# zzyunzhi/object-intrinsics

Measured on AMD Instinct MI355X. Metric: rendered rays/sec (64x64 img, 128 samples/ray) + D-images/sec, higher is better.
Workload: dtype f32 via f16x3 (fp32 operands split into 2 fp16 limbs = 22 mantissa bits, 3 fp16 MFMAs per product, fp32 accumulate: 2^-22 relative per product, 1e-4 parity path); 1 GPU; C2: 1x64x64 crop per GPU, 64+64 samples/ray, 1 up-sampling step(s), Generator.forward (render + Phong maps) + ADADiscriminatorView forward; parallelism=dp1 (independent renders, no data-path collective)

## Files before the change

object-intrinsics_amd/csrc/mlp_fwd3.hip:

```cpp
#include <type_traits>

#include "mlp_common.h"
#include "f3_blob.h"

namespace {

using namespace oimlp;
static_assert(oif3::FC == C && oif3::HB_SIG == H_SIG && oif3::HB_TABS_END == H_TABS_END && oif3::HB_BIAS == H_BIAS &&
              oif3::HB_WSCALE == H_WSCALE && oif3::HB_NL_SDF == NL_SDF, "f3_blob.h mirrors the packed header's offsets");

constexpr int F3_WAVES = 4;
constexpr int F3_TILE = F3_WAVES * WAVE_PTS;
using oif3::F3_FILM;
using oif3::F3_FILM_ROW;
using oif3::F3_TABS;
using oif3::F3_GMAX;
using oif3::F3_BLOB;
constexpr int F3_LDS = F3_BLOB + 2 * 65536;

typedef float Bank[16][4];
__device__ __forceinline__ float to_acc(float v) {
  float a;
  asm("v_accvgpr_write_b32 %0, %1" : "=a"(a) : "v"(v));
  return a;
}
__device__ __forceinline__ float from_acc(float a) {
  float v;
  asm("v_accvgpr_read_b32 %0, %1" : "=v"(v) : "a"(a));
  return v;
}

constexpr int F3_CU_SLOTS = 4096;
constexpr int F3_WG_SLOTS = 512;
__device__ __forceinline__ int cu_slot_id() {
  const unsigned xcc = __builtin_amdgcn_s_getreg((4 - 1) << 11 | 0 << 6 | 20);
  const unsigned cu = __builtin_amdgcn_s_getreg((8 - 1) << 11 | 8 << 6 | 4);
  return (int)(xcc * 256 + cu);
}

typedef float f32x2 __attribute__((ext_vector_type(2)));
__device__ __forceinline__ f32x2 pk_fma(f32x2 a, f32x2 b, f32x2 c) {
  return __builtin_elementwise_fma(a, b, c);
}
__device__ __forceinline__ f32x2 pk_mul(f32x2 a, f32x2 b) {
  return a * b;
}
__device__ __forceinline__ f32x2 pk_mul_s(f32x2 a, float s) {
  return a * s;
}
__device__ __forceinline__ f32x2 film_phase2(const f32x4& a, const f32x4& b, int k, float acc0, float acc1) {
  return pk_fma(f32x2{a[k], a[k + 1]}, f32x2{acc0, acc1}, f32x2{b[k], b[k + 1]});
}
__device__ __forceinline__ float max3_abs(float m, float x, float y) {
  float r;
  asm("v_max3_f32 %0, %1, |%2|, |%3|" : "=v"(r) : "v"(m), "v"(x), "v"(y));
  return r;
}

typedef unsigned Limbs[8][4];


__device__ __forceinline__ void split_limbs_normalised(const float (&act)[64], float m, float& run, Limbs& bh, Limbs& bl) {
  m = fmaxf(m, __shfl_xor(m, 32, 64));
  int eb = (__builtin_bit_cast(int, m) >> 23) & 0xff;
  eb = eb < 14 ? 14 : (eb > 254 ? 254 : eb);
  const float sc = __builtin_bit_cast(float, (267 - eb) << 23);
  run *= __builtin_bit_cast(float, (eb - 13) << 23);
#pragma unroll
  for (int s = 0; s < 8; ++s) {
#pragma unroll
    for (int d = 0; d < 4; ++d) split_pair(act[8 * s + 2 * d] * sc, act[8 * s + 2 * d + 1] * sc, bh[s][d], bl[s][d]);
    __builtin_amdgcn_sched_barrier(0);
  }
}
__device__ __forceinline__ void split_limbs(const float (&act)[64], Limbs& bh, Limbs& bl) {
#pragma unroll
  for (int s = 0; s < 8; ++s) {
#pragma unroll
    for (int d = 0; d < 4; ++d) split_pair(act[8 * s + 2 * d], act[8 * s + 2 * d + 1], bh[s][d], bl[s][d]);
    __builtin_amdgcn_sched_barrier(0);
  }
}

struct NoTail {
  __device__ __forceinline__ void operator()(int, int) const {}
};
template <class T> struct is_no_tail { static constexpr bool value = false; };
template <> struct is_no_tail<NoTail> { static constexpr bool value = true; };

constexpr int F3_ADIST = 1;
constexpr int F3_VALU_PER_MFMA = 6;
struct NoMid {
  __device__ __forceinline__ void operator()() const {}
};
template <class TAIL, class MID, class EPI>
__device__ __forceinline__ void stream_layer(const char* lds, const LayOff& y, const Limbs& bh, const Limbs& bl,
                                             f32x16 (&acc)[4], TAIL&& tail, MID&& mid, EPI&& epi) {
  constexpr bool HAS_TAIL = !is_no_tail<std::remove_cv_t<std::remove_reference_t<TAIL>>>::value;
  constexpr int AD = F3_ADIST;
  f32x4 ah[AD + 1], al[AD + 1];
#pragma unroll
  for (int i = 0; i < AD; ++i) {
    ah[i] = lds_f4(lds, i * 1024, y.wl);
    al[i] = lds_f4(lds, i * 1024, y.wh);
  }
#pragma unroll
  for (int t = 0; t < 4; ++t) {
#pragma unroll
    for (int r = 0; r < 16; ++r) acc[t][r] = 0.f;
#pragma unroll
    for (int s = 0; s < 8; ++s) {
      const int cur = t * 8 + s, nxt = cur + AD;
      if (nxt < 32) {
        ah[nxt % (AD + 1)] = lds_f4(lds, nxt * 1024, y.wl);
        al[nxt % (AD + 1)] = lds_f4(lds, nxt * 1024, y.wh);
      }
      int npairs = 0;
      if (t == 0) {
        if (HAS_TAIL && s < 6) {
          constexpr int first[7] = {0, 2, 3, 4, 6, 7, 8};
          for (int rp = first[s]; rp < first[s + 1]; ++rp) tail(3, rp);
          npairs = first[s + 1] - first[s];
        }
      } else {
        epi(t - 1, s);
        npairs = 1;
      }
      const int ci = cur % (AD + 1);
      const f16x8 wh = __builtin_bit_cast(f16x8, ah[ci]);
      const f16x8 wl = __builtin_bit_cast(f16x8, al[ci]);
      const u32x4 uh = {bh[s][0], bh[s][1], bh[s][2], bh[s][3]}, ul = {bl[s][0], bl[s][1], bl[s][2], bl[s][3]};
      const f16x8 vh = __builtin_bit_cast(f16x8, uh);
      const f16x8 vl = __builtin_bit_cast(f16x8, ul);
      acc[t] = __builtin_amdgcn_mfma_f32_32x32x16_f16(wl, vh, acc[t], 0, 0, 0);
      acc[t] = __builtin_amdgcn_mfma_f32_32x32x16_f16(wh, vl, acc[t], 0, 0, 0);
      acc[t] = __builtin_amdgcn_mfma_f32_32x32x16_f16(wh, vh, acc[t], 0, 0, 0);
      if (npairs >= 1) {
#pragma unroll
        for (int q = 0; q < 2; ++q) {
          __builtin_amdgcn_sched_group_barrier(0x008, 1, 0);
          if (npairs <= 1) __builtin_amdgcn_sched_group_barrier(0x002, F3_VALU_PER_MFMA, 0);
          else __builtin_amdgcn_sched_group_barrier(0x002, 2 * F3_VALU_PER_MFMA, 0);
        }
        __builtin_amdgcn_sched_group_barrier(0x008, 1, 0);
      }
      __builtin_amdgcn_sched_barrier(0);
    }
    if (t == 0) {
      mid();
      __builtin_amdgcn_sched_barrier(0);
    }
  }
}
template <class EPI>
__device__ __forceinline__ void run_tail(EPI&& epi) {
#pragma unroll
  for (int rp = 0; rp < 8; ++rp) {
    epi(3, rp);
    if (rp & 1) __builtin_amdgcn_sched_barrier(0);
  }
}

#ifdef OI_F3_PROF
__device__ unsigned long long oi_prof3[16];
#define F3_T(i)                                                  \
  do {                                                           \
    const unsigned long long t_ = __builtin_readcyclecounter();  \
    pacc[i] += t_ - tprev;                                       \
    tprev = t_;                                                  \
  } while (0)
#else
#define F3_T(i)
#endif

template <bool FAST>
__global__ void __launch_bounds__(64 * F3_WAVES) __attribute__((amdgpu_waves_per_eu(1, 1)))
sdf_mlp_full3_kernel(const float* __restrict__ pts, const char* __restrict__ packed, const float* __restrict__ gamma,
                     const float* __restrict__ beta, float* __restrict__ sdf_out, float* __restrict__ grad_out,
                     float* __restrict__ rgb_out, float* __restrict__ feat_out, char* __restrict__ scratch,
                     const char* __restrict__ blob, long long n_per_elem) {
  extern __shared__ __attribute__((aligned(16))) char lds[];
  constexpr int LB = 65536;
#ifdef OI_F3_PROF
  const unsigned long long t_entry = __builtin_readcyclecounter();
  const unsigned long long rt_entry = __builtin_amdgcn_s_memrealtime();
#endif
  const int tid = threadIdx.x, lane = tid & 63;
  const int wave = __builtin_amdgcn_readfirstlane(tid >> 6);
  const int h = lane >> 5, j = lane & 31;
  const int e = blockIdx.y;
  const float* hdr = reinterpret_cast<const float*>(packed);
  const char* mats = packed + H_BYTES;

  LaneOff o;
  o.h16 = 16 * h;
  o.h64 = 64 * h;
  o.l16 = 16 * lane;
  o.l16hi = 16 * lane + 32768;
  asm volatile("" : "+v"(o.h16), "+v"(o.h64), "+v"(o.l16), "+v"(o.l16hi));

  auto point_of = [&](bool& valid) {
    int jj = lane & 31;
    asm volatile("" : "+v"(jj));
    const long long local = (long long)blockIdx.x * F3_TILE + wave * WAVE_PTS + jj;
    valid = local < n_per_elem;
    return (long long)e * n_per_elem + (valid ? local : n_per_elem - 1);
  };

  FwdScratch<false> ws;
  {
    long long wg = (long long)e * gridDim.x + blockIdx.x;
    if ((long long)gridDim.x * gridDim.y > F3_WG_SLOTS) wg = cu_slot_id();
    ws.rs = __builtin_amdgcn_make_buffer_rsrc(scratch + (wg * F3_WAVES + wave) * 16384ll, 0, 16384, 0x00020000);
  }

  __amdgpu_buffer_rsrc_t feat_rs;
  int feat_off;
  {
    const long long base_pt = (long long)e * n_per_elem + (long long)blockIdx.x * F3_TILE + wave * WAVE_PTS;
    const long long left = n_per_elem - ((long long)blockIdx.x * F3_TILE + wave * WAVE_PTS);
    const int npts = feat_out == nullptr ? 0 : (left >= WAVE_PTS ? WAVE_PTS : (left > 0 ? (int)left : 0));
    feat_rs = __builtin_amdgcn_make_buffer_rsrc(feat_out + base_pt * C, 0, npts * C * 4, 0x00020000);
    feat_off = j * C * 4 + 16 * h;
  }

  const __amdgpu_buffer_rsrc_t img_rs =
      __builtin_amdgcn_make_buffer_rsrc(const_cast<char*>(mats), 0, NMAT * LB, 0x00020000);
  auto prefetch = [&](int pos) {
    const int m = pos < 7 ? pos : (pos < 12 ? 20 - pos : (pos < 14 ? pos - 12 : (pos < 16 ? 22 - pos : 14)));
#pragma unroll
    for (int q = 0; q < LB / 4096 / F3_WAVES; ++q) {
      const int c = (wave * (LB / 4096 / F3_WAVES) + q) * 4096;
      auto* dst = (__attribute__((address_space(3))) void*)(lds + F3_BLOB + (pos & 1) * LB + c);
      __builtin_amdgcn_raw_ptr_buffer_load_lds(img_rs, dst, 16, o.l16, m * LB + c, 0, 0);
      __builtin_amdgcn_raw_ptr_buffer_load_lds(img_rs, dst, 16, o.l16, m * LB + c, 1024, 0);
      __builtin_amdgcn_raw_ptr_buffer_load_lds(img_rs, dst, 16, o.l16, m * LB + c, 2048, 0);
      __builtin_amdgcn_raw_ptr_buffer_load_lds(img_rs, dst, 16, o.l16, m * LB + c, 3072, 0);
    }
  };
  auto lay = [&](int pos) {
    LayOff y;
    y.wl = o.l16 + F3_BLOB + (pos & 1) * LB;
    y.wh = y.wl + 32768;
    y.wq = 0;
    y.f16 = 0;
    return y;
  };
  auto film_base = [&](int l) { return o.h16 + F3_FILM + l * F3_FILM_ROW; };

  float px, py, pz;
  {
    bool valid;
    const long long pt = point_of(valid);
    px = pts[pt * 3 + 0], py = pts[pt * 3 + 1], pz = pts[pt * 3 + 2];
  }
  {
    const __amdgpu_buffer_rsrc_t blob_rs =
        __builtin_amdgcn_make_buffer_rsrc(const_cast<char*>(blob + (size_t)e * F3_BLOB), 0, F3_BLOB, 0x00020000);
#pragma unroll
    for (int q = 0; q < (F3_BLOB / 1024 + F3_WAVES - 1) / F3_WAVES; ++q) {
      const int c = q * F3_WAVES + wave;
      if (c < F3_BLOB / 1024)
        __builtin_amdgcn_raw_ptr_buffer_load_lds(blob_rs, (__attribute__((address_space(3))) void*)(lds + c * 1024), 16, o.l16,
                                                 c * 1024, 0, 0);
    }
  }
  prefetch(0);
  asm volatile("s_waitcnt vmcnt(%0) lgkmcnt(0)\n\ts_barrier" ::"n"(LB / 1024 / F3_WAVES) : "memory");
#ifdef OI_F3_PROF
  unsigned long long pacc[8] = {0, 0, 0, 0, 0, 0, 0, 0};
  unsigned long long tprev = __builtin_readcyclecounter();
  const unsigned long long tstart = tprev;
  pacc[4] = tstart - t_entry;
#endif
  float act[64];
  f32x16 acc[4];
  Limbs AH, AL, BH, BL;
  Bank P0, P1, P2, P3;
  struct Rows {
    f32x4 a, b, c, d;
  } rw[2];
  f32x4 fv;
  float run = 1.f, vmax = 0.f, sdf_part = 0.f;

  auto reduce = [&](float phi) { return FAST ? phi : __builtin_amdgcn_fractf(phi); };
  auto ld = [&](int imm, int base) { return lds_f4(lds, imm, base); };
#define ROW_A(FB, G) ld(grp_f0(G) * 4, FB)
#define ROW_B(FB, G) ld((C + grp_f0(G)) * 4, FB)
#define ROW_G(FB, G) ld((2 * C + grp_f0(G)) * 4, FB)
#define ROW_SIG(G) ld(F3_TABS + (H_SIG + grp_f0(G)) * 4, o.h16)

#define OI_PARK(BANK) [&](int g, int k, float r) { BANK[g][k] = to_acc(r); }
  auto no_park = [](int, int, float) {};

  auto layer0 = [&](Limbs& NH, Limbs& NL, auto&& park) {
    const int fb = film_base(0);
#pragma unroll
    for (int g = 0; g < 16; ++g) {
      const f32x4 a4 = ROW_A(fb, g), b4 = ROW_B(fb, g);
      float sn[4];
#pragma unroll
      for (int k = 0; k < 4; ++k) {
        const f32x4 w = lds_f4(lds, F3_TABS + H_TAB0 * 4 + (grp_f0(g) + k) * 16, o.h64);
        const float u = fmaf(pz, w[2], fmaf(py, w[1], px * w[0]));
        const float r = reduce(fmaf(a4[k], u, b4[k]));
        sn[k] = __builtin_amdgcn_sinf(r);
        park(g, k, r);
      }
      split_pair(sn[0], sn[1], NH[g >> 1][2 * (g & 1)], NL[g >> 1][2 * (g & 1)]);
      split_pair(sn[2], sn[3], NH[g >> 1][2 * (g & 1) + 1], NL[g >> 1][2 * (g & 1) + 1]);
      if (g & 1) __builtin_amdgcn_sched_barrier(0);
    }
  };

#define OI_FWD_EPI(FB, NH, NL, PARK, NEXT)                                                                 \
  [&](int tb, int rp) {                                                                                    \
    const int g = tb * 4 + (rp >> 1), k = 2 * (rp & 1);                                                    \
    Rows& R = rw[g & 1];                                                                                   \
    if (k == 0) {                                                                                          \
      if (g < 15) {                                                                                        \
        rw[(g + 1) & 1].a = ROW_A(FB, g + 1);                                                              \
        rw[(g + 1) & 1].b = ROW_B(FB, g + 1);                                                              \
      } else {                                                                                             \
        NEXT;                                                                                              \
      }                                                                                                    \
    }                                                                                                      \
    const f32x2 ph = film_phase2(R.a, R.b, k, acc[tb][2 * rp], acc[tb][2 * rp + 1]);                 \
    const float r0 = reduce(ph[0]), r1 = reduce(ph[1]);                                                    \
    PARK(g, k, r0);                                                                                        \
    PARK(g, k + 1, r1);                                                                                    \
    split_pair(__builtin_amdgcn_sinf(r0), __builtin_amdgcn_sinf(r1), NH[2 * tb + (rp >> 2)][rp & 3],       \
               NL[2 * tb + (rp >> 2)][rp & 3]);                                                            \
  }
  float sg = 1.f;
  auto pow2_for = [&](float U) {
    int eb = (__builtin_bit_cast(int, U) >> 23) & 0xff;
    eb = eb < 15 ? 15 : (eb > 253 ? 253 : eb);
    run *= __builtin_bit_cast(float, (eb - 14) << 23);
    sg = __builtin_bit_cast(float, (268 - eb) << 23);
  };
  const float* gmax = reinterpret_cast<const float*>(lds + F3_GMAX);
#define OI_REV_MID(L)                                                          \
  [&]() {                                                                      \
    const float m = fmaxf(vmax, __shfl_xor(vmax, 32, 64));                     \
    pow2_for(m * (hdr[H_BOUND + 6 + (L)] * gmax[(L)-1]));                      \
    vmax = 0.f;                                                                \
  }
#define OI_REV_EPI(FB, BANK, NH, NL, NEXT)                                                                 \
  [&](int tb, int rp) {                                                                                    \
    const int g = tb * 4 + (rp >> 1), k = 2 * (rp & 1);                                                    \
    Rows& R = rw[g & 1];                                                                                   \
    if (k == 0) {                                                                                          \
      if (g < 15) {                                                                                        \
        rw[(g + 1) & 1].c = ROW_G(FB, g + 1);                                                              \
      } else {                                                                                             \
        NEXT;                                                                                              \
      }                                                                                                    \
    }                                                                                                      \
    const f32x2 cs = {__builtin_amdgcn_cosf(from_acc(BANK[g][k])), __builtin_amdgcn_cosf(from_acc(BANK[g][k + 1]))};                     \
    const f32x2 v = pk_mul(pk_mul_s(f32x2{acc[tb][2 * rp], acc[tb][2 * rp + 1]}, sg),                \
                           pk_mul(f32x2{R.c[k], R.c[k + 1]}, cs));                                         \
    vmax = max3_abs(vmax, v[0], v[1]);                                                                     \
    split_pair(v[0], v[1], NH[2 * tb + (rp >> 2)][rp & 3], NL[2 * tb + (rp >> 2)][rp & 3]);                \
  }

  const LayOff y1 = lay(0), y2 = lay(1), y3 = lay(2), y4 = lay(3), y5 = lay(4), y6 = lay(5), y7 = lay(6);
  const int F0 = film_base(0), F1 = film_base(1), F2 = film_base(2), F3 = film_base(3), F4 = film_base(4),
            F5 = film_base(5), F6 = film_base(6), F7 = film_base(7), F8 = film_base(8), F9 = film_base(9);
#define NEXT_AB(FB) (rw[0].a = ROW_A(FB, 0), rw[0].b = ROW_B(FB, 0))
#define NEXT_G(FB) (rw[0].c = ROW_G(FB, 0))

  layer0(AH, AL, no_park);
  NEXT_AB(F1);
  F3_T(0);
  ring_sync();
  F3_T(2);
  prefetch(1);
  auto park0 = OI_PARK(P0);
  auto park1 = OI_PARK(P1);
  auto park2 = OI_PARK(P2);
  auto park3 = OI_PARK(P3);
  auto e1 = OI_FWD_EPI(F1, BH, BL, no_park, NEXT_AB(F2));
  stream_layer(lds, y1, AH, AL, acc, NoTail(), NoMid(), e1);
  F3_T(1);
  ring_sync();
  F3_T(2);
  prefetch(2);
  auto e2 = OI_FWD_EPI(F2, AH, AL, no_park, NEXT_AB(F3));
  stream_layer(lds, y2, BH, BL, acc, e1, NoMid(), e2);
  F3_T(1);
  ring_sync();
  F3_T(2);
  prefetch(3);
  auto e3 = OI_FWD_EPI(F3, BH, BL, park0, NEXT_AB(F4));
  stream_layer(lds, y3, AH, AL, acc, e2, NoMid(), e3);
  F3_T(1);
  ring_sync();
  F3_T(2);
  prefetch(4);
  auto e4 = OI_FWD_EPI(F4, AH, AL, park1, NEXT_AB(F5));
  stream_layer(lds, y4, BH, BL, acc, e3, NoMid(), e4);
  F3_T(1);
  ring_sync();
  F3_T(2);
  prefetch(5);
  auto e5 = OI_FWD_EPI(F5, BH, BL, park2, NEXT_AB(F6));
  stream_layer(lds, y5, AH, AL, acc, e4, NoMid(), e5);
  F3_T(1);
  ring_sync();
  F3_T(2);
  prefetch(6);
  auto e6 = OI_FWD_EPI(F6, AH, AL, park3,
                       (NEXT_AB(F7), rw[0].c = ROW_A(F9, 0), rw[0].d = ROW_SIG(0)));
  stream_layer(lds, y6, BH, BL, acc, e5, NoMid(), e6);
  F3_T(1);
  ring_sync();
  F3_T(2);
  prefetch(7);
  pow2_for(gmax[9] * 2.0f);
  const float sg7 = sg;
  auto e7 = [&](int tb, int rp) {
    const int g = tb * 4 + (rp >> 1), k = 2 * (rp & 1);
    Rows& R = rw[g & 1];
    if (k == 0) {
      if (g < 15) {
        Rows& N = rw[(g + 1) & 1];
        N.a = ROW_A(F7, g + 1);
        N.b = ROW_B(F7, g + 1);
        N.c = ROW_A(F9, g + 1);
        N.d = ROW_SIG(g + 1);
      } else {
        NEXT_G(F6);
      }
    }
    const f32x2 ph = film_phase2(R.a, R.b, k, acc[tb][2 * rp], acc[tb][2 * rp + 1]);
    f32x2 cs;
#pragma unroll
    for (int i = 0; i < 2; ++i) {
      const float r = reduce(ph[i]);
      const float sn = __builtin_amdgcn_sinf(r);
      fv[k + i] = sn;
      sdf_part = fmaf(sn, R.d[k + i], sdf_part);
      cs[i] = __builtin_amdgcn_cosf(r);
    }
    const f32x2 v = pk_mul(pk_mul_s(f32x2{R.c[k], R.c[k + 1]}, sg7), cs);
    vmax = max3_abs(vmax, v[0], v[1]);
    split_pair(v[0], v[1], BH[2 * tb + (rp >> 2)][rp & 3], BL[2 * tb + (rp >> 2)][rp & 3]);
    if (k == 2) {
      ws.store(0, g, o, fv);
      __builtin_amdgcn_raw_buffer_store_b128(__builtin_bit_cast(u32x4, fv), feat_rs, feat_off + grp_f0(g) * 4, 0, 0);
    }
  };
  stream_layer(lds, y7, AH, AL, acc, e6, NoMid(), e7);
  F3_T(1);
  ring_sync();
  F3_T(2);
  prefetch(8);

  auto r7 = OI_REV_EPI(F6, P3, AH, AL, NEXT_G(F5));
  stream_layer(lds, lay(7), BH, BL, acc, e7, OI_REV_MID(7), r7);
  {
    sdf_part += __shfl_xor(sdf_part, 32, 64);
    const float sdf_v = sdf_part + *reinterpret_cast<const float*>(lds + F3_TABS + (H_SIG + C) * 4);
    bool valid;
    const long long pt = point_of(valid);
    if (valid && h == 0) sdf_out[pt] = sdf_v;
  }
  F3_T(1);
  ring_sync();
  F3_T(2);
  prefetch(9);
  auto r6 = OI_REV_EPI(F5, P2, BH, BL, NEXT_G(F4));
  stream_layer(lds, lay(8), AH, AL, acc, r7, OI_REV_MID(6), r6);
  F3_T(1);
  ring_sync();
  F3_T(2);
  prefetch(10);
  auto r5 = OI_REV_EPI(F4, P1, AH, AL, NEXT_G(F3));
  stream_layer(lds, lay(9), BH, BL, acc, r6, OI_REV_MID(5), r5);
  F3_T(1);
  ring_sync();
  F3_T(2);
  prefetch(11);
  auto r4 = OI_REV_EPI(F3, P0, BH, BL, (void)0);
  stream_layer(lds, lay(10), AH, AL, acc, r5, OI_REV_MID(4), r4);
  F3_T(1);
  ring_sync();
  F3_T(2);
  prefetch(12);
  float one = 1.0f;
  asm volatile("" : "+v"(one));
  auto pg3 = [&](int tb, int rp) {
    const int g = tb * 4 + (rp >> 1), k = 2 * (rp & 1);
    const f32x2 a = pk_mul_s(f32x2{acc[tb][2 * rp], acc[tb][2 * rp + 1]}, one);
    vmax = max3_abs(vmax, a[0], a[1]);
    P0[g][k] = to_acc(a[0]);
    P0[g][k + 1] = to_acc(a[1]);
  };
  stream_layer(lds, lay(11), BH, BL, acc, r4, [&]() { vmax = 0.f; }, pg3);
  F3_T(1);
  ring_sync();
  F3_T(2);
  prefetch(13);
  run_tail(pg3);
  F3_T(3);

  const LayOff z1 = lay(12), z2 = lay(13);
  NEXT_AB(F1);
  layer0(AH, AL, park1);
  F3_T(0);
  auto f1 = OI_FWD_EPI(F1, BH, BL, park2, (NEXT_AB(F2), NEXT_G(F2)));
  stream_layer(lds, z1, AH, AL, acc, NoTail(), NoMid(), f1);
  F3_T(1);
  ring_sync();
  F3_T(2);
  prefetch(14);
  pow2_for(fmaxf(vmax, __shfl_xor(vmax, 32, 64)) * gmax[2]);
  vmax = 0.f;
  const float sg2 = sg;
  auto f2 = [&](int tb, int rp) {
    const int g = tb * 4 + (rp >> 1), k = 2 * (rp & 1);
    Rows& R = rw[g & 1];
    if (k == 0) {
      if (g < 15) {
        Rows& N = rw[(g + 1) & 1];
        N.a = ROW_A(F2, g + 1);
        N.b = ROW_B(F2, g + 1);
        N.c = ROW_G(F2, g + 1);
      } else {
        NEXT_G(F1);
      }
    }
    const f32x2 ph = film_phase2(R.a, R.b, k, acc[tb][2 * rp], acc[tb][2 * rp + 1]);
    const f32x2 cs = {__builtin_amdgcn_cosf(reduce(ph[0])), __builtin_amdgcn_cosf(reduce(ph[1]))};
    const f32x2 v = pk_mul(pk_mul_s(f32x2{from_acc(P0[g][k]), from_acc(P0[g][k + 1])}, sg2), pk_mul(f32x2{R.c[k], R.c[k + 1]}, cs));
    vmax = max3_abs(vmax, v[0], v[1]);
    split_pair(v[0], v[1], AH[2 * tb + (rp >> 2)][rp & 3], AL[2 * tb + (rp >> 2)][rp & 3]);
  };
  stream_layer(lds, z2, BH, BL, acc, f1, NoMid(), f2);
  F3_T(1);
  ring_sync();
  F3_T(2);
  prefetch(15);

  auto r2 = OI_REV_EPI(F1, P2, BH, BL, NEXT_G(F0));
  stream_layer(lds, lay(14), AH, AL, acc, f2, OI_REV_MID(2), r2);
  F3_T(1);
  ring_sync();
  F3_T(2);
  prefetch(16);
  auto r1 = [&](int tb, int rp) {
    const int g = tb * 4 + (rp >> 1), k = 2 * (rp & 1);
    Rows& R = rw[g & 1];
    if (k == 0 && g < 15) rw[(g + 1) & 1].c = ROW_G(F0, g + 1);
    const f32x2 cs = {__builtin_amdgcn_cosf(from_acc(P1[g][k])), __builtin_amdgcn_cosf(from_acc(P1[g][k + 1]))};
    const f32x2 v = pk_mul(f32x2{acc[tb][2 * rp], acc[tb][2 * rp + 1]}, pk_mul(f32x2{R.c[k], R.c[k + 1]}, cs));
    act[4 * g + k] = v[0];
    act[4 * g + k + 1] = v[1];
  };
  stream_layer(lds, lay(15), BH, BL, acc, r2, [&]() {}, r1);
  F3_T(1);
  run_tail(r1);
  F3_T(3);
  f32x4 fback[16];
#pragma unroll
  for (int g = 0; g < 16; ++g) fback[g] = ws.load(0, g, o);
  float gx = 0.f, gy = 0.f, gz = 0.f;
#pragma unroll
  for (int g = 0; g < 16; ++g) {
#pragma unroll
    for (int k = 0; k < 4; ++k) {
      const f32x4 w = lds_f4(lds, F3_TABS + H_TAB0 * 4 + (grp_f0(g) + k) * 16, o.h64);
      const float v = act[4 * g + k];
      gx = fmaf(v, w[0], gx);
      gy = fmaf(v, w[1], gy);
      gz = fmaf(v, w[2], gz);
    }
    if (g & 1) __builtin_amdgcn_sched_barrier(0);
  }
  gx += __shfl_xor(gx, 32, 64);
  gy += __shfl_xor(gy, 32, 64);
  gz += __shfl_xor(gz, 32, 64);
  gx *= run;
  gy *= run;
  gz *= run;
  bool valid;
  const long long pt = point_of(valid);
  if (valid && h == 0) {
    grad_out[pt * 3 + 0] = gx;
    grad_out[pt * 3 + 1] = gy;
    grad_out[pt * 3 + 2] = gz;
  }

  {
    ring_sync();
#pragma unroll
    for (int g = 0; g < 16; ++g)
#pragma unroll
      for (int k = 0; k < 4; ++k) act[4 * g + k] = fback[g][k];
    const LayOff yc = lay(16);
    const float cs3 = 1.0f / hdr[H_WSCALE + 14];
    const float vx = gx * cs3, vy = gy * cs3, vz = gz * cs3;
    float r0 = 0.f, r1 = 0.f, r2 = 0.f;
    f32x4 w0, w1, w2;
    split_limbs(act, AH, AL);
    NEXT_AB(F8);
    auto ec = [&](int tb, int rp) {
      const int g = tb * 4 + (rp >> 1), k = 2 * (rp & 1);
      Rows& R = rw[g & 1];
      if (k == 0) {
        if (g < 15) {
          rw[(g + 1) & 1].a = ROW_A(F8, g + 1);
          rw[(g + 1) & 1].b = ROW_B(F8, g + 1);
        }
        w0 = lds_f4(lds, F3_TABS + (H_RGB + 0 * C + grp_f0(g)) * 4, o.h16);
        w1 = lds_f4(lds, F3_TABS + (H_RGB + 1 * C + grp_f0(g)) * 4, o.h16);
        w2 = lds_f4(lds, F3_TABS + (H_RGB + 2 * C + grp_f0(g)) * 4, o.h16);
      }
#pragma unroll
      for (int i = 0; i < 2; ++i) {
        const f32x4 w = lds_f4(lds, F3_TABS + H_TABV * 4 + (grp_f0(g) + k + i) * 16, o.h64);
        const float u = acc[tb][2 * rp + i] + fmaf(vz, w[2], fmaf(vy, w[1], vx * w[0]));
        const float sn = __builtin_amdgcn_sinf(reduce(fmaf(R.a[k + i], u, R.b[k + i])));
        r0 = fmaf(sn, w0[k + i], r0);
        r1 = fmaf(sn, w1[k + i], r1);
        r2 = fmaf(sn, w2[k + i], r2);
      }
    };
    F3_T(5);
    stream_layer(lds, yc, AH, AL, acc, NoTail(), NoMid(), ec);
    F3_T(1);
    run_tail(ec);
    F3_T(3);
    r0 += __shfl_xor(r0, 32, 64);
    r1 += __shfl_xor(r1, 32, 64);
    r2 += __shfl_xor(r2, 32, 64);
    if (valid && h == 0 && rgb_out != nullptr) {
      const float* brgb = reinterpret_cast<const float*>(lds + F3_TABS + (H_RGB + 3 * C) * 4);
      rgb_out[pt * 3 + 0] = oi::sigmoidf_(r0 + brgb[0]);
      rgb_out[pt * 3 + 1] = oi::sigmoidf_(r1 + brgb[1]);
      rgb_out[pt * 3 + 2] = oi::sigmoidf_(r2 + brgb[2]);
    }
  }
#ifdef OI_F3_PROF
  F3_T(5);
  if (lane == 0) {
    for (int i = 0; i < 6; ++i) atomicAdd(&oi_prof3[i], pacc[i]);
    atomicAdd(&oi_prof3[6], __builtin_readcyclecounter() - tstart);
    atomicAdd(&oi_prof3[7], 1ull);
    atomicAdd(&oi_prof3[8], __builtin_readcyclecounter() - t_entry);
    atomicAdd(&oi_prof3[9], __builtin_amdgcn_s_memrealtime() - rt_entry);
  }
#endif
#undef OI_PARK
#undef OI_FWD_EPI
#undef OI_REV_EPI
#undef OI_REV_MID
#undef NEXT_AB
#undef NEXT_G
#undef ROW_A
#undef ROW_B
#undef ROW_G
#undef ROW_SIG
}

__global__ void __launch_bounds__(128) film_blob_f3_kernel(const char* __restrict__ packed, const float* __restrict__ gamma,
                                                           const float* __restrict__ beta, char* __restrict__ blob) {
  __shared__ float red[8];
  const int e = blockIdx.x, l = blockIdx.y, tid = threadIdx.x;
  const float* hdr = reinterpret_cast<const float*>(packed);
  float* out = reinterpret_cast<float*>(blob + (size_t)e * F3_BLOB);
  const float gm = tid < C ? gamma[((size_t)e * 9 + l) * C + tid] : 0.f, bt = tid < C ? beta[((size_t)e * 9 + l) * C + tid] : 0.f;
  oif3::blob_layer(hdr, out, l, tid, gm, bt, red);
}

size_t full3_slot_bytes(int B, long long n_per_elem) {
  const long long wgs = (long long)B * oi::cdiv(n_per_elem, F3_TILE);
  return (size_t)(wgs > F3_WG_SLOTS ? F3_CU_SLOTS : wgs) * F3_WAVES * 16384;
}

template <bool FAST>
int launch_full3(const float* pts, const char* pk, const float* gamma, const float* beta, float* sdf, float* grad,
                 float* rgb, float* feat, char* scratch, int B, long long n, bool blob_ready, hipStream_t st) {
  dim3 grid(oi::cdiv(n, F3_TILE), B), block(64 * F3_WAVES);
  auto k = sdf_mlp_full3_kernel<FAST>;
  (void)hipFuncSetAttribute(reinterpret_cast<const void*>(k), hipFuncAttributeMaxDynamicSharedMemorySize, F3_LDS);
  char* blob = scratch + full3_slot_bytes(B, n);
  if (!blob_ready) hipLaunchKernelGGL(film_blob_f3_kernel, dim3(B, 9), dim3(128), 0, st, pk, gamma, beta, blob);
  hipLaunchKernelGGL(k, grid, block, F3_LDS, st, pts, pk, gamma, beta, sdf, grad, rgb, feat, scratch, blob, n);
  return oi::check_launch("oi_sdf_mlp_fwd(full3)");
}

}

namespace oimlp {

size_t full3_scratch_bytes(int B, long long n_per_elem) {
  return full3_slot_bytes(B, n_per_elem) + (size_t)B * F3_BLOB;
}

size_t full3_blob_offset(int B, long long n_per_elem) { return full3_slot_bytes(B, n_per_elem); }

int launch_full3_f16x3(const float* pts, const void* packed, const float* gamma, const float* beta, float* sdf,
                       float* grad, float* rgb, float* feat, void* scratch, int B, long long n, int fast_trig, bool blob_ready,
                       hipStream_t st) {
  const char* pk = reinterpret_cast<const char*>(packed);
  char* sc = reinterpret_cast<char*>(scratch);
  return fast_trig ? launch_full3<true>(pts, pk, gamma, beta, sdf, grad, rgb, feat, sc, B, n, blob_ready, st)
                   : launch_full3<false>(pts, pk, gamma, beta, sdf, grad, rgb, feat, sc, B, n, blob_ready, st);
}

}

namespace {
__global__ void __launch_bounds__(256) cu_slot_selftest_kernel(int* busy, int* clashes, int* used, int spin) {
  extern __shared__ __attribute__((aligned(16))) char lds[];
  const int slot = cu_slot_id();
  if (threadIdx.x == 0) {
    if (atomicAdd(busy + slot, 1) != 0) atomicAdd(clashes, 1);
    atomicOr(used + slot, 1);
  }
  volatile float* l = reinterpret_cast<volatile float*>(lds);
  float acc = 0.f;
  for (int i = 0; i < spin; ++i) {
    l[threadIdx.x] = acc + i;
    acc += l[(threadIdx.x + 1) & 255];
  }
  __syncthreads();
  if (threadIdx.x == 0) {
    if (acc == 12345.678f) atomicAdd(clashes, 1 << 20);
    atomicAdd(busy + slot, -1);
  }
}
}

extern "C" int oi_selftest_cu_slots(int* busy, int* clashes, int* used, int n_workgroups, int spin, oi_stream_t stream) {
  OI_REQUIRE(busy && clashes && used && n_workgroups > 0, "oi_selftest_cu_slots: bad argument");
  auto k = cu_slot_selftest_kernel;
  (void)hipFuncSetAttribute(reinterpret_cast<const void*>(k), hipFuncAttributeMaxDynamicSharedMemorySize, F3_LDS);
  hipLaunchKernelGGL(k, dim3(n_workgroups), dim3(256), F3_LDS, oi::as_stream(stream), busy, clashes, used, spin);
  return oi::check_launch("oi_selftest_cu_slots");
}

#ifdef OI_F3_PROF
extern "C" int oi_prof3_read(unsigned long long* out, int reset) {
  (void)hipDeviceSynchronize();
  (void)hipMemcpyFromSymbol(out, HIP_SYMBOL(oi_prof3), sizeof(unsigned long long) * 16);
  if (reset) {
    unsigned long long z[16] = {0};
    (void)hipMemcpyToSymbol(HIP_SYMBOL(oi_prof3), z, sizeof(z));
  }
  return 0;
}
#endif
```

Before: 3.735 million rays/s.

## Park all six hidden-layer phases in packed AGPRs to skip forward recomputation

The fused SDF MLP forward+backward kernel previously stored phases for only four layers in AGPR banks. To backprop through layers 1-2 it recomputed them with a second forward pass, costing two extra weight-stream layers and extra prefetches. The new code truncates each phase to 21 bits and packs three values into two 32-bit AGPRs, so phases for all six layers fit and reverse mode runs straight through. Layer 0's phase is recomputed cheaply in the final reverse epilogue. The cost is extra bit-packing ALU work and reduced phase precision, which may affect the 1e-4 parity.

New measurement: 3.954 million rays/s (median of 6 runs). 1.06x the previous value.

```diff
diff --git a/object-intrinsics_amd/csrc/mlp_fwd3.hip b/object-intrinsics_amd/csrc/mlp_fwd3.hip
--- a/object-intrinsics_amd/csrc/mlp_fwd3.hip
+++ b/object-intrinsics_amd/csrc/mlp_fwd3.hip
@@ -18,16 +18,24 @@
 using oif3::F3_BLOB;
 constexpr int F3_LDS = F3_BLOB + 2 * 65536;
 
-typedef float Bank[16][4];
-__device__ __forceinline__ float to_acc(float v) {
-  float a;
+typedef unsigned Park[42];
+__device__ __forceinline__ unsigned to_acc(unsigned v) {
+  unsigned a;
   asm("v_accvgpr_write_b32 %0, %1" : "=a"(a) : "v"(v));
   return a;
 }
-__device__ __forceinline__ float from_acc(float a) {
-  float v;
+__device__ __forceinline__ unsigned from_acc(unsigned a) {
+  unsigned v;
   asm("v_accvgpr_read_b32 %0, %1" : "=v"(v) : "a"(a));
   return v;
+}
+__device__ __forceinline__ void pack3(unsigned ta, unsigned tb, unsigned tc, unsigned& d0, unsigned& d1) {
+  d0 = (ta << 11) | ((tc >> 10) & 0x7ffu);
+  d1 = (tb << 11) | (tc & 0x3ffu);
+}
+__device__ __forceinline__ unsigned unpack_ab(unsigned d, unsigned kx) { return __builtin_amdgcn_alignbit(kx, d, 9); }
+__device__ __forceinline__ unsigned unpack_c(unsigned d0, unsigned d1, unsigned kx) {
+  return __builtin_amdgcn_alignbit(kx, __builtin_amdgcn_alignbit(d0, d1 << 22, 11), 9);
 }
 
 constexpr int F3_CU_SLOTS = 4096;
@@ -227,7 +235,7 @@
   const __amdgpu_buffer_rsrc_t img_rs =
       __builtin_amdgcn_make_buffer_rsrc(const_cast<char*>(mats), 0, NMAT * LB, 0x00020000);
   auto prefetch = [&](int pos) {
-    const int m = pos < 7 ? pos : (pos < 12 ? 20 - pos : (pos < 14 ? pos - 12 : (pos < 16 ? 22 - pos : 14)));
+    const int m = pos < 7 ? pos : (pos < 14 ? 20 - pos : 14);
 #pragma unroll
     for (int q = 0; q < LB / 4096 / F3_WAVES; ++q) {
       const int c = (wave * (LB / 4096 / F3_WAVES) + q) * 4096;
@@ -276,7 +284,11 @@
   float act[64];
   f32x16 acc[4];
   Limbs AH, AL, BH, BL;
-  Bank P0, P1, P2, P3;
+  Park Q1, Q2, Q3, Q4, Q5, Q6;
+  unsigned XA0, XA1, XB0, XB1;
+  unsigned pq0 = 0, pq1 = 0;
+  unsigned kx = 0x7f;
+  asm volatile("" : "+s"(kx));
   struct Rows {
     f32x4 a, b, c, d;
   } rw[2];
@@ -290,47 +302,98 @@
 #define ROW_G(FB, G) ld((2 * C + grp_f0(G)) * 4, FB)
 #define ROW_SIG(G) ld(F3_TABS + (H_SIG + grp_f0(G)) * 4, o.h16)
 
-#define OI_PARK(BANK) [&](int g, int k, float r) { BANK[g][k] = to_acc(r); }
-  auto no_park = [](int, int, float) {};
-
-  auto layer0 = [&](Limbs& NH, Limbs& NL, auto&& park) {
+  auto park_fix = [&](float r) {
+    return __builtin_bit_cast(unsigned, (FAST ? __builtin_amdgcn_fractf(r) : r) + 4.0f);
+  };
+#define OI_PARK(Q, X0, X1, XPOS)                         \
+  [&](int p, float r0, float r1) {                       \
+    const unsigned t0 = park_fix(r0), t1 = park_fix(r1); \
+    unsigned d0, d1;                                     \
+    if (p % 3 == 0) {                                    \
+      pq0 = t0, pq1 = t1;                                \
+    } else if (p % 3 == 1) {                             \
+      pack3(pq0, pq1, t0, d0, d1);                       \
+      Q[4 * (p / 3)] = to_acc(d0);                       \
+      Q[4 * (p / 3) + 1] = to_acc(d1);                   \
+      if (p < 31) {                                      \
+        pq0 = t1;                                        \
+      } else if (XPOS == 0) {                            \
+        X0 = to_acc(t1);                                 \
+      } else if (XPOS == 1) {                            \
+        X1 = to_acc(t1);                                 \
+      } else {                                           \
+        pack3(from_acc(X0), from_acc(X1), t1, d0, d1);   \
+        X0 = to_acc(d0);                                 \
+        X1 = to_acc(d1);                                 \
+      }                                                  \
+    } else {                                             \
+      pack3(pq0, t0, t1, d0, d1);                        \
+      Q[4 * (p / 3) + 2] = to_acc(d0);                   \
+      Q[4 * (p / 3) + 3] = to_acc(d1);                   \
+    }                                                    \
+  }
+  auto no_park = [](int, float, float) {};
+#define OI_UNPARK(Q, X0, X1, XPOS)                     \
+  [&](int p, unsigned& x0, unsigned& x1) {             \
+    if (p % 3 == 0) {                                  \
+      pq0 = from_acc(Q[4 * (p / 3)]);                  \
+      pq1 = from_acc(Q[4 * (p / 3) + 1]);              \
+      x0 = unpack_ab(pq0, kx);                         \
+      x1 = unpack_ab(pq1, kx);                         \
+    } else if (p % 3 == 1) {                           \
+      x0 = unpack_c(pq0, pq1, kx);                     \
+      if (p < 31) {                                    \
+        pq0 = from_acc(Q[4 * (p / 3) + 2]);            \
+        x1 = unpack_ab(pq0, kx);                       \
+      } else if (XPOS == 0) {                          \
+        x1 = unpack_ab(from_acc(X0), kx);              \
+      } else if (XPOS == 1) {                          \
+        x1 = unpack_ab(from_acc(X1), kx);              \
+      } else {                                         \
+        x1 = unpack_c(from_acc(X0), from_acc(X1), kx); \
+      }                                                \
+    } else {                                           \
+      pq1 = from_acc(Q[4 * (p / 3) + 3]);              \
+      x0 = unpack_ab(pq1, kx);                         \
+      x1 = unpack_c(pq0, pq1, kx);                     \
+    }                                                  \
+  }
+
+  auto tab0_row = [&](int f) { return lds_f4(lds, F3_TABS + H_TAB0 * 4 + f * 16, o.h64); };
+  auto phase0 = [&](const f32x4& w, float a, float b) {
+    return reduce(fmaf(a, fmaf(pz, w[2], fmaf(py, w[1], px * w[0])), b));
+  };
+  auto layer0 = [&](Limbs& NH, Limbs& NL) {
     const int fb = film_base(0);
 #pragma unroll
     for (int g = 0; g < 16; ++g) {
       const f32x4 a4 = ROW_A(fb, g), b4 = ROW_B(fb, g);
       float sn[4];
 #pragma unroll
-      for (int k = 0; k < 4; ++k) {
-        const f32x4 w = lds_f4(lds, F3_TABS + H_TAB0 * 4 + (grp_f0(g) + k) * 16, o.h64);
-        const float u = fmaf(pz, w[2], fmaf(py, w[1], px * w[0]));
-        const float r = reduce(fmaf(a4[k], u, b4[k]));
-        sn[k] = __builtin_amdgcn_sinf(r);
-        park(g, k, r);
-      }
+      for (int k = 0; k < 4; ++k) sn[k] = __builtin_amdgcn_sinf(phase0(tab0_row(grp_f0(g) + k), a4[k], b4[k]));
       split_pair(sn[0], sn[1], NH[g >> 1][2 * (g & 1)], NL[g >> 1][2 * (g & 1)]);
       split_pair(sn[2], sn[3], NH[g >> 1][2 * (g & 1) + 1], NL[g >> 1][2 * (g & 1) + 1]);
       if (g & 1) __builtin_amdgcn_sched_barrier(0);
     }
   };
 
-#define OI_FWD_EPI(FB, NH, NL, PARK, NEXT)                                                                 \
-  [&](int tb, int rp) {                                                                                    \
-    const int g = tb * 4 + (rp >> 1), k = 2 * (rp & 1);                                                    \
-    Rows& R = rw[g & 1];                                                                                   \
-    if (k == 0) {                                                                                          \
-      if (g < 15) {                                                                                        \
-        rw[(g + 1) & 1].a = ROW_A(FB, g + 1);                                                              \
-        rw[(g + 1) & 1].b = ROW_B(FB, g + 1);                                                              \
-      } else {                                                                                             \
-        NEXT;                                                                                              \
-      }                                                                                                    \
-    }                                                                                                      \
+#define OI_FWD_EPI(FB, NH, NL, PARK, NEXT)                                                           \
+  [&](int tb, int rp) {                                                                              \
+    const int g = tb * 4 + (rp >> 1), k = 2 * (rp & 1);                                              \
+    Rows& R = rw[g & 1];                                                                             \
+    if (k == 0) {                                                                                    \
+      if (g < 15) {                                                                                  \
+        rw[(g + 1) & 1].a = ROW_A(FB, g + 1);                                                        \
+        rw[(g + 1) & 1].b = ROW_B(FB, g + 1);                                                        \
+      } else {                                                                                       \
+        NEXT;                                                                                        \
+      }                                                                                              \
+    }                                                                                                \
     const f32x2 ph = film_phase2(R.a, R.b, k, acc[tb][2 * rp], acc[tb][2 * rp + 1]);                 \
-    const float r0 = reduce(ph[0]), r1 = reduce(ph[1]);                                                    \
-    PARK(g, k, r0);                                                                                        \
-    PARK(g, k + 1, r1);                                                                                    \
-    split_pair(__builtin_amdgcn_sinf(r0), __builtin_amdgcn_sinf(r1), NH[2 * tb + (rp >> 2)][rp & 3],       \
-               NL[2 * tb + (rp >> 2)][rp & 3]);                                                            \
+    const float r0 = reduce(ph[0]), r1 = reduce(ph[1]);                                              \
+    PARK(tb * 8 + rp, r0, r1);                                                                       \
+    split_pair(__builtin_amdgcn_sinf(r0), __builtin_amdgcn_sinf(r1), NH[2 * tb + (rp >> 2)][rp & 3], \
+               NL[2 * tb + (rp >> 2)][rp & 3]);                                                      \
   }
   float sg = 1.f;
   auto pow2_for = [&](float U) {
@@ -340,28 +403,31 @@
     sg = __builtin_bit_cast(float, (268 - eb) << 23);
   };
   const float* gmax = reinterpret_cast<const float*>(lds + F3_GMAX);
-#define OI_REV_MID(L)                                                          \
-  [&]() {                                                                      \
-    const float m = fmaxf(vmax, __shfl_xor(vmax, 32, 64));                     \
-    pow2_for(m * (hdr[H_BOUND + 6 + (L)] * gmax[(L)-1]));                      \
-    vmax = 0.f;                                                                \
-  }
-#define OI_REV_EPI(FB, BANK, NH, NL, NEXT)                                                                 \
-  [&](int tb, int rp) {                                                                                    \
-    const int g = tb * 4 + (rp >> 1), k = 2 * (rp & 1);                                                    \
-    Rows& R = rw[g & 1];                                                                                   \
-    if (k == 0) {                                                                                          \
-      if (g < 15) {                                                                                        \
-        rw[(g + 1) & 1].c = ROW_G(FB, g + 1);                                                              \
-      } else {                                                                                             \
-        NEXT;                                                                                              \
-      }                                                                                                    \
-    }                                                                                                      \
-    const f32x2 cs = {__builtin_amdgcn_cosf(from_acc(BANK[g][k])), __builtin_amdgcn_cosf(from_acc(BANK[g][k + 1]))};                     \
-    const f32x2 v = pk_mul(pk_mul_s(f32x2{acc[tb][2 * rp], acc[tb][2 * rp + 1]}, sg),                \
-                           pk_mul(f32x2{R.c[k], R.c[k + 1]}, cs));                                         \
-    vmax = max3_abs(vmax, v[0], v[1]);                                                                     \
-    split_pair(v[0], v[1], NH[2 * tb + (rp >> 2)][rp & 3], NL[2 * tb + (rp >> 2)][rp & 3]);                \
+#define OI_REV_MID(L)                                      \
+  [&]() {                                                  \
+    const float m = fmaxf(vmax, __shfl_xor(vmax, 32, 64)); \
+    pow2_for(m * (hdr[H_BOUND + 6 + (L)] * gmax[(L)-1]));  \
+    vmax = 0.f;                                            \
+  }
+#define OI_REV_EPI(FB, UNPARK, NH, NL, NEXT)                                                \
+  [&](int tb, int rp) {                                                                     \
+    const int g = tb * 4 + (rp >> 1), k = 2 * (rp & 1);                                     \
+    Rows& R = rw[g & 1];                                                                    \
+    if (k == 0) {                                                                           \
+      if (g < 15) {                                                                         \
+        rw[(g + 1) & 1].c = ROW_G(FB, g + 1);                                               \
+      } else {                                                                              \
+        NEXT;                                                                               \
+      }                                                                                     \
+    }                                                                                       \
+    unsigned x0, x1;                                                                        \
+    UNPARK(tb * 8 + rp, x0, x1);                                                            \
+    const f32x2 cs = {__builtin_amdgcn_cosf(__builtin_bit_cast(float, x0)),                 \
+                      __builtin_amdgcn_cosf(__builtin_bit_cast(float, x1))};                \
+    const f32x2 v = pk_mul(pk_mul_s(f32x2{acc[tb][2 * rp], acc[tb][2 * rp + 1]}, sg),       \
+                           pk_mul(f32x2{R.c[k], R.c[k + 1]}, cs));                          \
+    vmax = max3_abs(vmax, v[0], v[1]);                                                      \
+    split_pair(v[0], v[1], NH[2 * tb + (rp >> 2)][rp & 3], NL[2 * tb + (rp >> 2)][rp & 3]); \
   }
 
   const LayOff y1 = lay(0), y2 = lay(1), y3 = lay(2), y4 = lay(3), y5 = lay(4), y6 = lay(5), y7 = lay(6);
@@ -370,47 +436,49 @@
 #define NEXT_AB(FB) (rw[0].a = ROW_A(FB, 0), rw[0].b = ROW_B(FB, 0))
 #define NEXT_G(FB) (rw[0].c = ROW_G(FB, 0))
 
-  layer0(AH, AL, no_park);
+  layer0(AH, AL);
   NEXT_AB(F1);
   F3_T(0);
   ring_sync();
   F3_T(2);
   prefetch(1);
-  auto park0 = OI_PARK(P0);
-  auto park1 = OI_PARK(P1);
-  auto park2 = OI_PARK(P2);
-  auto park3 = OI_PARK(P3);
-  auto e1 = OI_FWD_EPI(F1, BH, BL, no_park, NEXT_AB(F2));
+  auto park1 = OI_PARK(Q1, XA0, XA1, 0);
+  auto park2 = OI_PARK(Q2, XA0, XA1, 1);
+  auto park3 = OI_PARK(Q3, XA0, XA1, 2);
+  auto park4 = OI_PARK(Q4, XB0, XB1, 0);
+  auto park5 = OI_PARK(Q5, XB0, XB1, 1);
+  auto park6 = OI_PARK(Q6, XB0, XB1, 2);
+  auto e1 = OI_FWD_EPI(F1, BH, BL, park1, NEXT_AB(F2));
   stream_layer(lds, y1, AH, AL, acc, NoTail(), NoMid(), e1);
   F3_T(1);
   ring_sync();
   F3_T(2);
   prefetch(2);
-  auto e2 = OI_FWD_EPI(F2, AH, AL, no_park, NEXT_AB(F3));
+  auto e2 = OI_FWD_EPI(F2, AH, AL, park2, NEXT_AB(F3));
   stream_layer(lds, y2, BH, BL, acc, e1, NoMid(), e2);
   F3_T(1);
   ring_sync();
   F3_T(2);
   prefetch(3);
-  auto e3 = OI_FWD_EPI(F3, BH, BL, park0, NEXT_AB(F4));
+  auto e3 = OI_FWD_EPI(F3, BH, BL, park3, NEXT_AB(F4));
   stream_layer(lds, y3, AH, AL, acc, e2, NoMid(), e3);
   F3_T(1);
   ring_sync();
   F3_T(2);
   prefetch(4);
-  auto e4 = OI_FWD_EPI(F4, AH, AL, park1, NEXT_AB(F5));
+  auto e4 = OI_FWD_EPI(F4, AH, AL, park4, NEXT_AB(F5));
   stream_layer(lds, y4, BH, BL, acc, e3, NoMid(), e4);
   F3_T(1);
   ring_sync();
   F3_T(2);
   prefetch(5);
-  auto e5 = OI_FWD_EPI(F5, BH, BL, park2, NEXT_AB(F6));
+  auto e5 = OI_FWD_EPI(F5, BH, BL, park5, NEXT_AB(F6));
   stream_layer(lds, y5, AH, AL, acc, e4, NoMid(), e5);
   F3_T(1);
   ring_sync();
   F3_T(2);
   prefetch(6);
-  auto e6 = OI_FWD_EPI(F6, AH, AL, park3,
+  auto e6 = OI_FWD_EPI(F6, AH, AL, park6,
                        (NEXT_AB(F7), rw[0].c = ROW_A(F9, 0), rw[0].d = ROW_SIG(0)));
   stream_layer(lds, y6, BH, BL, acc, e5, NoMid(), e6);
   F3_T(1);
@@ -457,7 +525,13 @@
   F3_T(2);
   prefetch(8);
 
-  auto r7 = OI_REV_EPI(F6, P3, AH, AL, NEXT_G(F5));
+  auto un6 = OI_UNPARK(Q6, XB0, XB1, 2);
+  auto un5 = OI_UNPARK(Q5, XB0, XB1, 1);
+  auto un4 = OI_UNPARK(Q4, XB0, XB1, 0);
+  auto un3 = OI_UNPARK(Q3, XA0, XA1, 2);
+  auto un2 = OI_UNPARK(Q2, XA0, XA1, 1);
+  auto un1 = OI_UNPARK(Q1, XA0, XA1, 0);
+  auto r7 = OI_REV_EPI(F6, un6, AH, AL, NEXT_G(F5));
   stream_layer(lds, lay(7), BH, BL, acc, e7, OI_REV_MID(7), r7);
   {
     sdf_part += __shfl_xor(sdf_part, 32, 64);
@@ -470,95 +544,59 @@
   ring_sync();
   F3_T(2);
   prefetch(9);
-  auto r6 = OI_REV_EPI(F5, P2, BH, BL, NEXT_G(F4));
+  auto r6 = OI_REV_EPI(F5, un5, BH, BL, NEXT_G(F4));
   stream_layer(lds, lay(8), AH, AL, acc, r7, OI_REV_MID(6), r6);
   F3_T(1);
   ring_sync();
   F3_T(2);
   prefetch(10);
-  auto r5 = OI_REV_EPI(F4, P1, AH, AL, NEXT_G(F3));
+  auto r5 = OI_REV_EPI(F4, un4, AH, AL, NEXT_G(F3));
   stream_layer(lds, lay(9), BH, BL, acc, r6, OI_REV_MID(5), r5);
   F3_T(1);
   ring_sync();
   F3_T(2);
   prefetch(11);
-  auto r4 = OI_REV_EPI(F3, P0, BH, BL, (void)0);
+  auto r4 = OI_REV_EPI(F3, un3, BH, BL, NEXT_G(F2));
   stream_layer(lds, lay(10), AH, AL, acc, r5, OI_REV_MID(4), r4);
   F3_T(1);
   ring_sync();
   F3_T(2);
   prefetch(12);
-  float one = 1.0f;
-  asm volatile("" : "+v"(one));
-  auto pg3 = [&](int tb, int rp) {
-    const int g = tb * 4 + (rp >> 1), k = 2 * (rp & 1);
-    const f32x2 a = pk_mul_s(f32x2{acc[tb][2 * rp], acc[tb][2 * rp + 1]}, one);
-    vmax = max3_abs(vmax, a[0], a[1]);
-    P0[g][k] = to_acc(a[0]);
-    P0[g][k + 1] = to_acc(a[1]);
-  };
-  stream_layer(lds, lay(11), BH, BL, acc, r4, [&]() { vmax = 0.f; }, pg3);
+  auto r3 = OI_REV_EPI(F2, un2, AH, AL, NEXT_G(F1));
+  stream_layer(lds, lay(11), BH, BL, acc, r4, OI_REV_MID(3), r3);
   F3_T(1);
   ring_sync();
   F3_T(2);
   prefetch(13);
-  run_tail(pg3);
-  F3_T(3);
-
-  const LayOff z1 = lay(12), z2 = lay(13);
-  NEXT_AB(F1);
-  layer0(AH, AL, park1);
-  F3_T(0);
-  auto f1 = OI_FWD_EPI(F1, BH, BL, park2, (NEXT_AB(F2), NEXT_G(F2)));
-  stream_layer(lds, z1, AH, AL, acc, NoTail(), NoMid(), f1);
+  f32x4 wq0, wq1;
+  auto r2 = OI_REV_EPI(F1, un1, BH, BL,
+                       (NEXT_AB(F0), NEXT_G(F0), wq0 = tab0_row(grp_f0(0)), wq1 = tab0_row(grp_f0(0) + 1)));
+  stream_layer(lds, lay(12), AH, AL, acc, r3, OI_REV_MID(2), r2);
   F3_T(1);
   ring_sync();
   F3_T(2);
   prefetch(14);
-  pow2_for(fmaxf(vmax, __shfl_xor(vmax, 32, 64)) * gmax[2]);
-  vmax = 0.f;
-  const float sg2 = sg;
-  auto f2 = [&](int tb, int rp) {
-    const int g = tb * 4 + (rp >> 1), k = 2 * (rp & 1);
-    Rows& R = rw[g & 1];
-    if (k == 0) {
-      if (g < 15) {
-        Rows& N = rw[(g + 1) & 1];
-        N.a = ROW_A(F2, g + 1);
-        N.b = ROW_B(F2, g + 1);
-        N.c = ROW_G(F2, g + 1);
-      } else {
-        NEXT_G(F1);
-      }
-    }
-    const f32x2 ph = film_phase2(R.a, R.b, k, acc[tb][2 * rp], acc[tb][2 * rp + 1]);
-    const f32x2 cs = {__builtin_amdgcn_cosf(reduce(ph[0])), __builtin_amdgcn_cosf(reduce(ph[1]))};
-    const f32x2 v = pk_mul(pk_mul_s(f32x2{from_acc(P0[g][k]), from_acc(P0[g][k + 1])}, sg2), pk_mul(f32x2{R.c[k], R.c[k + 1]}, cs));
-    vmax = max3_abs(vmax, v[0], v[1]);
-    split_pair(v[0], v[1], AH[2 * tb + (rp >> 2)][rp & 3], AL[2 * tb + (rp >> 2)][rp & 3]);
-  };
-  stream_layer(lds, z2, BH, BL, acc, f1, NoMid(), f2);
-  F3_T(1);
-  ring_sync();
-  F3_T(2);
-  prefetch(15);
-
-  auto r2 = OI_REV_EPI(F1, P2, BH, BL, NEXT_G(F0));
-  stream_layer(lds, lay(14), AH, AL, acc, f2, OI_REV_MID(2), r2);
-  F3_T(1);
-  ring_sync();
-  F3_T(2);
-  prefetch(16);
   auto r1 = [&](int tb, int rp) {
     const int g = tb * 4 + (rp >> 1), k = 2 * (rp & 1);
     Rows& R = rw[g & 1];
-    if (k == 0 && g < 15) rw[(g + 1) & 1].c = ROW_G(F0, g + 1);
-    const f32x2 cs = {__builtin_amdgcn_cosf(from_acc(P1[g][k])), __builtin_amdgcn_cosf(from_acc(P1[g][k + 1]))};
+    if (k == 0 && g < 15) {
+      rw[(g + 1) & 1].a = ROW_A(F0, g + 1);
+      rw[(g + 1) & 1].b = ROW_B(F0, g + 1);
+      rw[(g + 1) & 1].c = ROW_G(F0, g + 1);
+    }
+    const f32x4 w0 = wq0, w1 = wq1;
+    if (tb * 8 + rp < 31) {
+      const int gn = tb * 4 + ((rp + 1) >> 1), kn = 2 * ((rp + 1) & 1);
+      wq0 = tab0_row(grp_f0(gn) + kn);
+      wq1 = tab0_row(grp_f0(gn) + kn + 1);
+    }
+    const f32x2 cs = {__builtin_amdgcn_cosf(phase0(w0, R.a[k], R.b[k])),
+                      __builtin_amdgcn_cosf(phase0(w1, R.a[k + 1], R.b[k + 1]))};
     const f32x2 v = pk_mul(f32x2{acc[tb][2 * rp], acc[tb][2 * rp + 1]}, pk_mul(f32x2{R.c[k], R.c[k + 1]}, cs));
     act[4 * g + k] = v[0];
     act[4 * g + k + 1] = v[1];
   };
-  stream_layer(lds, lay(15), BH, BL, acc, r2, [&]() {}, r1);
+  stream_layer(lds, lay(13), BH, BL, acc, r2, [&]() {}, r1);
   F3_T(1);
   run_tail(r1);
   F3_T(3);
@@ -598,7 +636,7 @@
     for (int g = 0; g < 16; ++g)
 #pragma unroll
       for (int k = 0; k < 4; ++k) act[4 * g + k] = fback[g][k];
-    const LayOff yc = lay(16);
+    const LayOff yc = lay(14);
     const float cs3 = 1.0f / hdr[H_WSCALE + 14];
     const float vx = gx * cs3, vy = gy * cs3, vz = gz * cs3;
     float r0 = 0.f, r1 = 0.f, r2 = 0.f;
@@ -653,6 +691,7 @@
   }
 #endif
 #undef OI_PARK
+#undef OI_UNPARK
 #undef OI_FWD_EPI
 #undef OI_REV_EPI
 #undef OI_REV_MID
```
